# wmtlab/tactileSR

Measured on AMD Instinct MI355X. Metric: SR samples/sec (4x4->40x40), higher is better.
Workload: dtype f32 as 2 power-of-two-scaled fp16 planes x 3 MFMA products, fp32 accumulate (fp32-grade); 1 GPU; tactileSR_model eval forward 4x4->40x40, batch=4096/GPU, fp32 in/out (BASELINE configs[1]); batch_per_gpu=4096, scale_factor=10, seqsCnt=1, parallelism=replicas x1, conv_impl=fp16x3, dist_world_size=1

## Files before the change

### tactilesr_amd/csrc/conv_mfma_k32.hip

```cpp
#include "tsr_common.h"
#include "conv_args.h"
#include "conv_epilogue16.h"
#include "conv_fuse1x1_16.h"
#include "conv_host.h"
#include "tactilesr_hip.h"
#include <type_traits>

typedef _Float16 kf16x8 __attribute__((ext_vector_type(8)));
typedef _Float16 kf16x4 __attribute__((ext_vector_type(4)));

constexpr int k32_row_slots(int px) {
  int rs = px * 4;
  while ((rs & 3) != 2) ++rs;
  return rs;
}

template <int KS, int COUT, int WN, bool DBH = false, int NTHR = 256> struct K32Geom {
  static constexpr int IMG = (NTHR / 64) / WN;
  static constexpr int HH = 8 + KS - 1;
  static constexpr int T = KS * KS;
  static constexpr int HS = (T - 1) / 2;
  static constexpr int PIXB = 64;
  static constexpr int ROWB = k32_row_slots(HH) * 16;
  static constexpr int IMGB = HH * ROWB;
  static constexpr int HALO_B = IMG * IMGB;
  static constexpr int SROWB = k32_row_slots(8) * 16;
  static constexpr int SIMGB = 8 * SROWB;
  static constexpr int SIDE_B = DBH ? 0 : IMG * SIMGB;
  static constexpr int WTAP_B = 2 * 16 * COUT * 2;
  static constexpr int WSLAB_B = 2 * WTAP_B;
  static constexpr int NHB = DBH ? 2 : 1;
  static constexpr int MAIN_LDS = NHB * HALO_B + SIDE_B + 3 * WSLAB_B;
};

constexpr int PAIR_KH[12] = {0, 0, 0, 2, 1, 3, 4, 4, 1, 1, 2, 3};
constexpr int PAIR_KW[12] = {0, 2, 4, 4, 0, 0, 1, 3, 1, 3, 1, 1};
constexpr int PAIR_V[12] = {0, 0, 1, 1, 1, 1, 0, 0, 0, 1, 0, 0};
constexpr int PAIR_OUTER = 8;

template <int KS, int COUT, bool EXT, int WN, bool FUSE2 = false, bool DBH = false, int NTHR = 256, bool PAIR = false>
__global__ __launch_bounds__(NTHR, NTHR == 512 ? 1 : 2) void conv_k32_kernel(const ConvArgs a) {
  static_assert(!PAIR || (KS == 5 && COUT == 128 && !EXT && !FUSE2 && !DBH), "pair form: 5x5 geometry, inference");
  static_assert(COUT == 64 * WN, "every wave owns 64 channels");
  static_assert(!FUSE2 || (!EXT && COUT == 128), "fused 1x1: 128 channels, inference");
  static_assert(NTHR == 256 || (NTHR == 512 && WN == 2), "512 threads: 4 images x 2 C_out halves");
  typedef K32Geom<KS, COUT, WN, DBH, NTHR> G;
  constexpr int NW = NTHR / 64;
  constexpr bool WDMA = !EXT;
  constexpr int IMG = G::IMG, P = KS / 2, HH = G::HH, T = G::T, HS = G::HS, NT = COUT / (16 * WN);
  constexpr int PIXB = G::PIXB, ROWB = G::ROWB, IMGB = G::IMGB, HALO_B = G::HALO_B;
  constexpr int SROWB = G::SROWB, SIMGB = G::SIMGB, SIDE_B = G::SIDE_B;
  constexpr int WTAP_B = G::WTAP_B, WSLAB_B = G::WSLAB_B;
  constexpr int WITEMS = WSLAB_B / 16, WV = (WITEMS + NTHR - 1) / NTHR;
  constexpr int NITEM = IMG * HH * HH * 4, NIT = (NITEM + NTHR - 1) / NTHR;
  constexpr int FUSE_LDS = FUSE2 ? Fuse1x1Geom16<IMG>::BYTES + 64 : 0;
  __shared__ __attribute__((aligned(16))) char lds[G::MAIN_LDS > FUSE_LDS ? G::MAIN_LDS : FUSE_LDS];
  char* halo = lds;
  char* wbuf = lds + G::NHB * HALO_B + SIDE_B;

  const int tid = threadIdx.x;
  const int lane = tid & 63;
  const int wave = tid >> 6;
  const int wave_s = __builtin_amdgcn_readfirstlane(wave);
  const int wm = WN == 2 ? wave >> 1 : wave, wn = WN == 2 ? wave & 1 : 0;
  const int m = lane & 15, g = lane >> 4, khalf = g & 1, tsel = g >> 1;

  float sx = 1.f, accmul = 1.f, sxh = 1.f;
  int bid;
  {
    const int nwg = gridDim.x, q = nwg >> 3, r = nwg & 7;
    const int xcd = blockIdx.x & 7, idx = blockIdx.x >> 3;
    bid = (xcd < r ? xcd * (q + 1) : r * (q + 1) + (xcd - r) * q) + idx;
  }
  const int tpi = a.tiles_x * a.tiles_y;
  const int ig = bid / tpi;
  const int trem = bid - ig * tpi;
  const int ebase = bid * IMG;
  const int ty = trem / a.tiles_x, tx = trem - ty * a.tiles_x;
  const int y0 = ty * 8, x0 = tx * 8, b0 = ig * IMG;
  const int HW = a.H * a.W;
  const int in_blocks = a.in_ctot >> 4;

  int st_src[NIT], st_dst[NIT];
#pragma unroll
  for (int k = 0; k < NIT; ++k) {
    const int it = tid + k * NTHR;
    st_src[k] = -1;
    st_dst[k] = -1;
    if (it < NITEM) {
      const int qd = it & 3, px = it >> 2;
      const int img = px / (HH * HH), rem = px - img * (HH * HH);
      const int hy = rem / HH, hx = rem - hy * HH;
      const int gy = y0 - P + hy, gx = x0 - P + hx, b = b0 + img;
      st_dst[k] = img * IMGB + hy * ROWB + hx * PIXB + qd * 8;
      if (b < a.B && gy >= 0 && gy < a.H && gx >= 0 && gx < a.W)
        st_src[k] = ((img * in_blocks) * HW + gy * a.W + gx) * 16 + qd * 4;
    }
  }
  const float* in_base = a.in + ((size_t)b0 * in_blocks + (a.in_coff >> 4)) * HW * 16;

  const int laneA0 = wm * IMGB + (m >> 3) * ROWB + (m & 7) * PIXB + khalf * 16;
  const int lx = laneA0 + tsel * PIXB;
  constexpr int CK = PAIR ? 3 : KS - 1;
  const int lw = PAIR ? laneA0 + tsel * ROWB
                      : laneA0 + tsel * (ROWB - (KS - 1) * PIXB);
  const int lc = tsel ? laneA0 + CK * ROWB + CK * PIXB
                      : HALO_B + wm * SIMGB + (m >> 3) * SROWB + (m & 7) * PIXB + khalf * 16;
  const int lcs = tsel ? 2 * ROWB : 2 * SROWB;
  const int lcd = laneA0 + (KS - 1) * (ROWB + PIXB) + tsel * HALO_B;
  const int laneB = tsel * WTAP_B + (khalf * COUT + wn * (COUT / WN) + m) * 16;
  const int laneBh = tsel * (WTAP_B / 2) + (khalf * 64 + wn * 32 + m) * 16;

  f32x4 acc[4][NT];
#pragma unroll
  for (int mt = 0; mt < 4; ++mt)
#pragma unroll
    for (int nt = 0; nt < NT; ++nt) acc[mt][nt] = (f32x4){0.f, 0.f, 0.f, 0.f};

  const int nreal = a.cin >> 4;
  const int nchunk = nreal + (nreal & 1);
  const int S = (nchunk >> 1) * T;
  const char* wsrc = (const char*)a.wp;
  const __amdgpu_buffer_rsrc_t wrsrc = __builtin_amdgcn_make_buffer_rsrc((void*)a.wp, 0, 0x7fffffff, 0x00020000);

  f32x4 hsc = {1.f, 1.f, 1.f, 1.f}, hsh = {0.f, 0.f, 0.f, 0.f};
  auto load_halo = [&](int c, f32x4* hv) __attribute__((always_inline)) {
    const float* inc = in_base + (size_t)(c < nreal ? c : nreal - 1) * HW * 16;
    if (EXT && a.in_scale) {
      const int cq = (c < nreal ? c : nreal - 1) * 16 + (tid & 3) * 4;
      hsc = *(const f32x4*)(a.in_scale + cq);
      hsh = *(const f32x4*)(a.in_shift + cq);
    }
#pragma unroll
    for (int k = 0; k < NIT; ++k) hv[k] = *(const f32x4*)(inc + (unsigned)(st_src[k] < 0 ? 0 : st_src[k]));
  };
  auto store_halo = [&](const f32x4* hv, int c, int hb = 0) __attribute__((always_inline)) {
#pragma unroll
    for (int k = 0; k < NIT; ++k) {
      if (st_dst[k] >= 0) {
        f32x4 v = hv[k];
        if (EXT && a.in_scale) {
#pragma unroll
          for (int jj = 0; jj < 4; ++jj) v[jj] = tsr_relu_x2(fmaf(v[jj], hsc[jj], hsh[jj]));
        }
        const bool inside = st_src[k] >= 0 && c < nreal;
#pragma unroll
        for (int jj = 0; jj < 4; ++jj) v[jj] = inside ? v[jj] * sxh : 0.f;
#pragma unroll
        for (int p = 0; p < 2; ++p) {
          kf16x4 bq;
#pragma unroll
          for (int jj = 0; jj < 4; ++jj) {
            bq[jj] = (_Float16)v[jj];
            v[jj] -= (float)bq[jj];
          }
          *(kf16x4*)(halo + hb * HALO_B + st_dst[k] + p * 32) = bq;
        }
      }
    }
  };
#define DMA_BYTES(goff_, slot_, nv_)                                                     \
  {                                                                                      \
    const int vo_ = (int)(goff_) + tid * 16;                                             \
    char* dst_ = wbuf + (slot_) * WSLAB_B + wave_s * 1024;                               \
    _Pragma("unroll") for (int v = 0; v < (nv_); ++v)                                    \
      __builtin_amdgcn_raw_ptr_buffer_load_lds(wrsrc, (__attribute__((address_space(3))) void*)(dst_ + v * NTHR * 16), 16, \
                                               vo_ + v * NTHR * 16, 0, 0, 0);             \
  }
#define LOAD_W(sidx)                                                                     \
  {                                                                                      \
    const f32x4* src_ = (const f32x4*)(wsrc + (size_t)(sidx) * WSLAB_B);                  \
    _Pragma("unroll") for (int v = 0; v < WV; ++v) wreg[v] = src_[tid + v * NTHR];        \
  }
#define STORE_W(slot)                                                                    \
  {                                                                                      \
    char* wb_ = wbuf + (slot) * WSLAB_B;                                                 \
    _Pragma("unroll") for (int v = 0; v < WV; ++v) ((f32x4*)wb_)[tid + v * NTHR] = wreg[v]; \
  }
#define DMA_W(sidx, slot) DMA_BYTES((size_t)(sidx) * WSLAB_B, slot, WV)
#define DMA_WAIT_N(n_) __builtin_amdgcn_s_waitcnt(0x0F70 | ((n_) & 15) | (((n_) >> 4) << 14))
#define DMA_WAIT() DMA_WAIT_N(0)
#define PAIR_HALF(pq_) ((pq_) < 24 && ((pq_) % 12) < PAIR_OUTER)
#define DMA_WP(slot, pq_)                                                                \
  {                                                                                      \
    if (PAIR_HALF(pq_)) { DMA_BYTES(woff, slot, WV / 2); woff += WSLAB_B / 2; }          \
    else { DMA_BYTES(woff, slot, WV); woff += WSLAB_B; }                                 \
  }
#define STEP_BARRIER() __syncthreads()
#define LOAD_A(dst, p_, st_, hb_)                                                        \
  {                                                                                      \
    const int kh_ = PAIR ? PAIR_KH[(st_)] : (2 * (st_)) / KS, kw_ = PAIR ? PAIR_KW[(st_)] : (2 * (st_)) - kh_ * KS; \
    const bool x_ = PAIR ? PAIR_V[(st_)] == 0 : kw_ < KS - 1;                            \
    const char* ab_ = lds + (x_ ? lx : lw) + (hb_) * HALO_B + kh_ * ROWB + kw_ * PIXB + (p_) * 32; \
    _Pragma("unroll") for (int mt = 0; mt < 4; ++mt) dst[mt] = *(const kf16x8*)(ab_ + mt * 2 * ROWB); \
  }
#define LOAD_A_CROSS(dst, p_)                                                            \
  {                                                                                      \
    _Pragma("unroll") for (int mt = 0; mt < 4; ++mt) dst[mt] = *(const kf16x8*)(lds + lc + mt * lcs + (p_) * 32); \
  }
#define LOAD_A_CROSSD(dst, p_)                                                           \
  {                                                                                      \
    _Pragma("unroll") for (int mt = 0; mt < 4; ++mt) dst[mt] = *(const kf16x8*)(lds + lcd + mt * 2 * ROWB + (p_) * 32); \
  }
#define LOAD_B(dst, p_, slot_)                                                           \
  {                                                                                      \
    const char* wb_ = wbuf + (slot_) * WSLAB_B + laneB + (p_) * (2 * COUT * 16);         \
    _Pragma("unroll") for (int nt = 0; nt < NT; ++nt) dst[nt] = *(const kf16x8*)(wb_ + nt * 256); \
  }
#define LOAD_B_HI(dst, p_, slot_)                                                        \
  {                                                                                      \
    const char* wb_ = wbuf + (slot_) * WSLAB_B + laneBh + (p_) * (2 * 64 * 16);          \
    _Pragma("unroll") for (int nt = 2; nt < NT; ++nt) dst[nt] = *(const kf16x8*)(wb_ + (nt - 2) * 256); \
  }
#define MFMA_PHASE_HI(A_, B_)                                                            \
  _Pragma("unroll") for (int mt = 0; mt < 4; ++mt)                                       \
    _Pragma("unroll") for (int nt = 2; nt < NT; ++nt)                                    \
      acc[mt][nt] = __builtin_amdgcn_mfma_f32_16x16x32_f16(A_[mt], B_[nt], acc[mt][nt], 0, 0, 0);
#define MFMA_PHASE(A_, B_)                                                               \
  _Pragma("unroll") for (int mt = 0; mt < 4; ++mt)                                       \
    _Pragma("unroll") for (int nt = 0; nt < NT; ++nt)                                    \
      acc[mt][nt] = __builtin_amdgcn_mfma_f32_16x16x32_f16(A_[mt], B_[nt], acc[mt][nt], 0, 0, 0);
#define INTERLEAVE(n_, per_)                                                             \
  _Pragma("unroll") for (int i_ = 0; i_ < (n_); ++i_) {                                  \
    __builtin_amdgcn_sched_group_barrier(0x008, (per_), 0);                              \
    __builtin_amdgcn_sched_group_barrier(0x100, 1, 0);                                   \
  }

  auto operand_scales = [&]() __attribute__((always_inline)) {
    float mx = a.in_amax ? *a.in_amax : 0.f;
    if (EXT && a.in_scale) {
      __shared__ float bnd[2 * NW];
      float ms = 0.f, mt = 0.f;
      for (int c = threadIdx.x; c < a.cin; c += NTHR) {
        ms = fmaxf(ms, fabsf(a.in_scale[c]));
        mt = fmaxf(mt, fabsf(a.in_shift[c]));
      }
#pragma unroll
      for (int o = 32; o > 0; o >>= 1) {
        ms = fmaxf(ms, __shfl_xor(ms, o));
        mt = fmaxf(mt, __shfl_xor(mt, o));
      }
      if (lane == 0) { bnd[wave * 2] = ms; bnd[wave * 2 + 1] = mt; }
      __syncthreads();
      ms = 0.f; mt = 0.f;
#pragma unroll
      for (int w = 0; w < NW; ++w) { ms = fmaxf(ms, bnd[2 * w]); mt = fmaxf(mt, bnd[2 * w + 1]); }
      mx = mx * ms + mt;
    }
    if (mx > 0.f) {
      int e = (int)((__float_as_uint(mx) >> 23) & 0xFF) - 127;
      int be = 13 - e + 127;
      be = be < 1 ? 1 : (be > 254 ? 254 : be);
      sx = __uint_as_float((unsigned)be << 23);
    }
    float w_inv = a.w_inv_scale;
    if (a.w_amax) {
      const float wmx = *a.w_amax;
      w_inv = 1.f;
      if (wmx > 0.f && wmx < 3.0e38f) {
        int be = 127 - (13 - ((int)((__float_as_uint(wmx) >> 23) & 0xFF) - 127));
        be = be < 1 ? 1 : (be > 254 ? 254 : be);
        w_inv = __uint_as_float((unsigned)be << 23);
      }
    }
    accmul = w_inv / sx;
    sxh = (EXT && a.in_scale) ? 0.5f * sx : sx;
  };

  f32x4 hv[NIT], wreg[WDMA ? 1 : WV];
  size_t woff = 0;
  load_halo(0, hv);
  if constexpr (PAIR) {
    DMA_WP(0, 0);
    DMA_WP(1, 1);
    operand_scales();
  } else if constexpr (WDMA) {
    DMA_W(0, 0);
    if (S > 1) DMA_W(1, 1);
    operand_scales();
  } else {
    LOAD_W(0);
    operand_scales();
    STORE_W(0);
    if (S > 1) { LOAD_W(1); STORE_W(1); }
  }
  store_halo(hv, 0);
  if constexpr (WDMA) { DMA_WAIT(); } else { if (S > 2) LOAD_W(2); }
  __syncthreads();

  kf16x8 A0[4], A1[4], B0[NT] = {}, B1[NT] = {};
  LOAD_A(A1, 1, 0, 0);
  if constexpr (PAIR) { LOAD_B_HI(B0, 0, 0); } else { LOAD_B(B0, 0, 0); }

  constexpr int SCI = IMG * 256 / NTHR, SCS = NTHR / 256;
  const int sc_t = tid & 255, sc_i0 = tid >> 8;
  const int sc_src = sc_i0 * IMGB + ((sc_t >> 5) + CK) * ROWB + (((sc_t >> 2) & 7) + CK) * PIXB + (sc_t & 3) * 16;
  const int sc_dst = HALO_B + sc_i0 * SIMGB + (sc_t >> 5) * SROWB + ((sc_t >> 2) & 7) * PIXB + (sc_t & 3) * 16;

  int s = 0;
  int slot = 0;
  auto block = [&](int c, auto oddc) __attribute__((always_inline)) {
    constexpr int ODD = decltype(oddc)::value;
    constexpr int NST = HS + ODD;
#pragma unroll
    for (int st = 0; st < NST; ++st) {
      const int slot1 = slot == 2 ? 0 : slot + 1;
      const int slot2 = slot1 == 2 ? 0 : slot1 + 1;
      const bool cross = ODD && st == HS;
      f32x4 sidev[SCI];
      if (WDMA && s + 2 < S) {
        if constexpr (PAIR) { DMA_WP(slot2, (ODD * HS + st + 2) % 25); } else { DMA_W(s + 2, slot2); }
      }
      const bool outer = PAIR && st < PAIR_OUTER;
      const bool next_outer = PAIR && (st + 1 < PAIR_OUTER || st + 1 == NST);
      if (cross) { LOAD_A_CROSS(A0, 0); } else { LOAD_A(A0, 0, st, 0); }
      if (outer) { LOAD_B_HI(B1, 1, slot); } else { LOAD_B(B1, 1, slot); }
      if (!ODD && st == 0) {
#pragma unroll
        for (int k = 0; k < SCI; ++k) sidev[k] = *(const f32x4*)(lds + sc_src + k * SCS * IMGB);
      }
      if (st == NST - 2 && c + 1 < nchunk) load_halo(c + 1, hv);
      if (outer) {
        MFMA_PHASE_HI(A1, B0);
        if (!ODD && st == 0) { INTERLEAVE(6 + SCI, 1); } else { INTERLEAVE(6, 1); }
      } else {
        MFMA_PHASE(A1, B0);
        if (!ODD && st == 0) { INTERLEAVE(8 + SCI, 1); } else { INTERLEAVE(8, 2); }
      }
      if (st + 1 < NST) {
        if (ODD && st + 1 == HS) { LOAD_A_CROSS(A1, 1); } else { LOAD_A(A1, 1, st + 1, 0); }
      }
      if (outer) {
        MFMA_PHASE_HI(A0, B0);
        if (st + 1 < NST) { INTERLEAVE(4, 2); }
      } else {
        MFMA_PHASE(A0, B0);
        if (st + 1 < NST) { INTERLEAVE(4, 4); }
      }
      if (next_outer) { LOAD_B_HI(B0, 0, slot1); } else { LOAD_B(B0, 0, slot1); }
      if (outer) {
        MFMA_PHASE_HI(A0, B1);
        if (next_outer) { INTERLEAVE(2, 4); } else { INTERLEAVE(4, 2); }
      } else {
        MFMA_PHASE(A0, B1);
        if (next_outer) { INTERLEAVE(2, 8); } else { INTERLEAVE(4, 4); }
      }
      if (!ODD && st == 0) {
#pragma unroll
        for (int k = 0; k < SCI; ++k) *(f32x4*)(lds + sc_dst + k * SCS * SIMGB) = sidev[k];
      }
      if constexpr (WDMA) {
        if (st == NST - 2 && c + 1 < nchunk) { DMA_WAIT_N(NIT); } else { DMA_WAIT(); }
      } else {
        if (s + 2 < S) STORE_W(slot2);
        if (s + 3 < S) LOAD_W(s + 3);
      }
      STEP_BARRIER();
      if (st + 1 == NST && c + 1 < nchunk) {
        store_halo(hv, c + 1);
        __syncthreads();
        LOAD_A(A1, 1, 0, 0);
      }
      ++s;
      slot = slot1;
    }
  };
  if constexpr (!DBH) {
    for (int c = 0; c < nchunk; c += 2) {
      block(c, std::integral_constant<int, 0>());
      block(c + 1, std::integral_constant<int, 1>());
    }
  } else {
    for (int c = 0; c < nchunk; c += 2) {
#pragma unroll
      for (int p = 0; p < T; ++p) {
        const int slot1 = slot == 2 ? 0 : slot + 1;
        const int slot2 = slot1 == 2 ? 0 : slot1 + 1;
        if (WDMA && s + 2 < S) DMA_W(s + 2, slot2);
        if (p == HS) { LOAD_A_CROSSD(A0, 0); }
        else if (p < HS) { LOAD_A(A0, 0, p, 0); }
        else { LOAD_A(A0, 0, p - HS - 1, 1); }
        LOAD_B(B1, 1, slot);
        if (p == 0) load_halo(c + 1, hv);
        if (p == HS + 1 && c + 2 < nchunk) load_halo(c + 2, hv);
        MFMA_PHASE(A1, B0);
        INTERLEAVE(8, 2);
        if (p + 1 == HS) { LOAD_A_CROSSD(A1, 1); }
        else if (p + 1 < HS) { LOAD_A(A1, 1, p + 1, 0); }
        else if (p + 1 < T) { LOAD_A(A1, 1, p - HS, 1); }
        else { LOAD_A(A1, 1, 0, 0); }
        MFMA_PHASE(A0, B0);
        INTERLEAVE(4, 4);
        LOAD_B(B0, 0, slot1);
        MFMA_PHASE(A0, B1);
        INTERLEAVE(4, 4);
        if (p == HS - 2) store_halo(hv, c + 1, 1);
        if (p == T - 2 && c + 2 < nchunk) store_halo(hv, c + 2, 0);
        if constexpr (WDMA) {
          if (p == 0 || (p == HS + 1 && c + 2 < nchunk)) { DMA_WAIT_N(NIT); } else { DMA_WAIT(); }
        } else {
          if (s + 2 < S) STORE_W(slot2);
          if (s + 3 < S) LOAD_W(s + 3);
        }
        STEP_BARRIER();
        ++s;
        slot = slot1;
      }
    }
  }
#undef DMA_W
#undef LOAD_W
#undef STORE_W
#undef DMA_WP
#undef DMA_BYTES
#undef DMA_WAIT
#undef DMA_WAIT_N
#undef PAIR_HALF
#undef STEP_BARRIER
#undef LOAD_A
#undef LOAD_A_CROSS
#undef LOAD_A_CROSSD
#undef LOAD_B
#undef LOAD_B_HI
#undef MFMA_PHASE_HI
#undef MFMA_PHASE
#undef INTERLEAVE

  if constexpr (FUSE2) conv_fuse1x1_epilogue16<IMG>(a, acc, lds, b0, y0, x0, wm, wn, lane, HW, accmul);
  else conv_epilogue16<COUT, EXT, WN>(a, acc, ebase, b0, y0, x0, wm, wn, lane, HW, accmul);
}

int tsr_conv_k32_images(int cout) { (void)cout; return 4; }

template <int KS, int COUT, bool EXT>
static int launch_k32(const ConvArgs& a, hipStream_t st) {
  constexpr int WN = COUT / 64;
  if constexpr (COUT == 128 && EXT) {
    const int grid = ((a.B + 3) / 4) * a.tiles_x * a.tiles_y;
    hipLaunchKernelGGL((conv_k32_kernel<KS, COUT, EXT, WN, false, KS == 3, 512>), dim3(grid), dim3(512), 0, st, a);
    return tsr_check_launch();
  }
  constexpr int IMG = 4 / WN;
  const int grid = ((a.B + IMG - 1) / IMG) * a.tiles_x * a.tiles_y;
  hipLaunchKernelGGL((conv_k32_kernel<KS, COUT, EXT, WN, false, KS == 3>), dim3(grid), dim3(256), 0, st, a);
  return tsr_check_launch();
}

template <bool EXT> static int dispatch_k32(const ConvArgs& a, int cout, int ks, hipStream_t st) {
  return for_cout_ks(cout, ks, [&](auto CO, auto KS) {
    if constexpr (decltype(KS)::value > 1) return launch_k32<decltype(KS)::value, decltype(CO)::value, EXT>(a, st);
    else return (int)TSR_ERR_ARG;
  });
}
int tsr_conv_k32(const ConvArgs& a, int cout, int ks, bool ext, hipStream_t st) {
  return ext ? dispatch_k32<true>(a, cout, ks, st) : dispatch_k32<false>(a, cout, ks, st);
}

__host__ __device__ inline int pair_logical_channel(int k) {
  const int wn = k >> 6, nt = (k >> 4) & 3, c = k & 15;
  return (nt < 2 ? 0 : 64) + wn * 32 + (nt & 1) * 16 + c;
}
extern "C" int tsr_pair_channel_perm(int* perm128) {
  if (!perm128) return TSR_ERR_ARG;
  for (int k = 0; k < 128; ++k) perm128[k] = pair_logical_channel(k);
  return TSR_OK;
}

__global__ void pack_pair_kernel(const float* __restrict__ w3, const float* __restrict__ w5, _Float16* __restrict__ wp,
                                 int cin, float wscale, const float* __restrict__ w_amax) {
  if (w_amax) {
    const float wm = *w_amax;
    wscale = 1.f;
    if (wm > 0.f && wm < 3.0e38f) {
      int be = 127 + 13 - ((int)((__float_as_uint(wm) >> 23) & 0xFF) - 127);
      be = be < 1 ? 1 : (be > 254 ? 254 : be);
      wscale = __uint_as_float((unsigned)be << 23);
    }
  }
  const int cin_p = (cin + 31) & ~31;
  const size_t total = (size_t)128 * cin_p * 25;
  for (size_t i = blockIdx.x * (size_t)blockDim.x + threadIdx.x; i < total; i += (size_t)gridDim.x * blockDim.x) {
    const int j = i & 7;
    size_t r = i >> 3;
    const int k = r & 127; r >>= 7;
    const int kh2 = r & 1; r >>= 1;
    const int tap = r % 25;
    const int chunk = r / 25;
    const int ci = chunk * 16 + kh2 * 8 + j;
    const int kh = tap / 5, kw = tap - kh * 5;
    const int nt = (k >> 4) & 3, ch = (k >> 6) * 32 + (nt & 1) * 16 + (k & 15);
    float v = 0.f;
    if (ci < cin) {
      if (nt >= 2) v = w5[((size_t)ch * cin + ci) * 25 + tap];
      else if (kh >= 1 && kh <= 3 && kw >= 1 && kw <= 3) v = w3[((size_t)ch * cin + ci) * 9 + (kh - 1) * 3 + (kw - 1)];
    }
    v *= wscale;
    int pos = 24;
#pragma unroll
    for (int st = 0; st < 12; ++st) {
      if (kh == PAIR_KH[st] && kw == PAIR_KW[st]) pos = 2 * st;
      if (kh == PAIR_KH[st] + PAIR_V[st] && kw == PAIR_KW[st] + 1 - PAIR_V[st]) pos = 2 * st + 1;
    }
    const int odd = chunk & 1;
    const bool half = pos < 2 * PAIR_OUTER;
    if (half && nt < 2) continue;
    size_t base = (size_t)(chunk >> 1) * (2 * 65536 + 8192);
    if (pos >= 24) base += 2 * 65536 + (size_t)odd * 4096;
    else if (half) base += (size_t)odd * 65536 + (size_t)(pos >> 1) * 4096 + (size_t)(pos & 1) * 2048;
    else base += (size_t)odd * 65536 + 32768 + (size_t)((pos - 16) >> 1) * 8192 + (size_t)(pos & 1) * 4096;
    const int nch = half ? 64 : 128;
    const int kk = half ? (k >> 6) * 32 + (nt - 2) * 16 + (k & 15) : k;
    for (int p = 0; p < 2; ++p) {
      const _Float16 q = (_Float16)v;
      v -= (float)q;
      wp[base + ((size_t)(p * 2 + kh2) * nch + kk) * 8 + j] = q;
    }
  }
}

extern "C" long long tsr_conv_weight_pair_elems(int cin) { return (long long)(((cin + 31) & ~31) / 32) * (2 * 65536 + 8192); }

extern "C" int tsr_pack_conv_weight_pair_f16s(const float* w3_oihw, const float* w5_oihw, void* w_packed, int cin,
                                              float wscale, const float* w_amax, void* stream) {
  if (!w3_oihw || !w5_oihw || !w_packed || cin <= 0 || (cin & 15) || (!w_amax && !(wscale > 0.f))) return TSR_ERR_ARG;
  hipLaunchKernelGGL(pack_pair_kernel, pack_grid((size_t)128 * ((cin + 31) & ~31) * 25), dim3(256), 0, (hipStream_t)stream,
                     w3_oihw, w5_oihw, (_Float16*)w_packed, cin, wscale, w_amax);
  return tsr_check_launch();
}

extern "C" int tsr_conv2d_fwd_f16s_pair(const float* in, int in_ctot, int in_coff, int cin, const void* w_packed,
                                        float w_inv_scale, const float* in_amax, float* out_amax,
                                        const float* scale, const float* shift, float* out, int out_ctot, int out_coff,
                                        int relu, int B, int H, int W, void* stream) {
  ConvArgs a;
  if (!f16s_scales_ok(in_amax, w_inv_scale) ||
      conv_fill(a, in, in_ctot, in_coff, cin, w_packed, scale, shift, nullptr, 0, 0, out, out_ctot, out_coff, 128, relu, B, H, W))
    return TSR_ERR_ARG;
  a.in_amax = in_amax; a.w_inv_scale = w_inv_scale; a.out_amax = out_amax;
  const int grid = ((B + 1) / 2) * a.tiles_x * a.tiles_y;
  hipLaunchKernelGGL((conv_k32_kernel<5, 128, false, 2, false, false, 256, true>), dim3(grid), dim3(256), 0,
                     (hipStream_t)stream, a);
  return tsr_check_launch();
}

int tsr_conv_k32_fuse1x1(const ConvArgs& a, int ks, hipStream_t st) {
  const int grid = ((a.B + 1) / 2) * a.tiles_x * a.tiles_y;
  if (ks == 5) hipLaunchKernelGGL((conv_k32_kernel<5, 128, false, 2, true>), dim3(grid), dim3(256), 0, st, a);
  else hipLaunchKernelGGL((conv_k32_kernel<3, 128, false, 2, true, true>), dim3(grid), dim3(256), 0, st, a);
  return tsr_check_launch();
}
```

Before: 31830 samples/s.

## Interleave per-row MFMA with split LDS and weight-DMA loads for 5x5 convs

For the non-paired DMA path with 5x5 kernels, the step loop is restructured so each MFMA row is issued alongside individual A/B fragment LDS reads and individual weight DMA pieces, with explicit sched_group_barrier hints per row. The aim is to hide LDS and global-to-LDS latency behind matrix work instead of issuing loads in bulk phases. The buffer resource is also given a tight byte bound instead of a huge range, so the prefetch issued past the last step (it is no longer guarded by s+2<S) reads out of range and returns zero rather than touching memory. This adds scheduling complexity and relies on the bounds check, and the hand-tuned order may hurt if the compiler's own interleave was already better.

```diff
diff --git a/tactilesr_amd/csrc/conv_mfma_k32.hip b/tactilesr_amd/csrc/conv_mfma_k32.hip
--- a/tactilesr_amd/csrc/conv_mfma_k32.hip
+++ b/tactilesr_amd/csrc/conv_mfma_k32.hip
@@ -121,7 +121,8 @@
   const int nchunk = nreal + (nreal & 1);
   const int S = (nchunk >> 1) * T;
   const char* wsrc = (const char*)a.wp;
-  const __amdgpu_buffer_rsrc_t wrsrc = __builtin_amdgcn_make_buffer_rsrc((void*)a.wp, 0, 0x7fffffff, 0x00020000);
+  const int wbytes = !WDMA ? 0x7fffffff : PAIR ? (nchunk >> 1) * ((2 * 65536 + 8192) * 2) : S * WSLAB_B;
+  const __amdgpu_buffer_rsrc_t wrsrc = __builtin_amdgcn_make_buffer_rsrc((void*)a.wp, 0, wbytes, 0x00020000);
 
   f32x4 hsc = {1.f, 1.f, 1.f, 1.f}, hsh = {0.f, 0.f, 0.f, 0.f};
   auto load_halo = [&](int c, f32x4* hv) __attribute__((always_inline)) {
@@ -167,6 +168,9 @@
       __builtin_amdgcn_raw_ptr_buffer_load_lds(wrsrc, (__attribute__((address_space(3))) void*)(dst_ + v * NTHR * 16), 16, \
                                                vo_ + v * NTHR * 16, 0, 0, 0);             \
   }
+#define DMA_PIECE(vo_, slot_, v_)                                                        \
+  __builtin_amdgcn_raw_ptr_buffer_load_lds(wrsrc, (__attribute__((address_space(3))) void*)(wbuf + (slot_) * WSLAB_B + wave_s * 1024 + (v_) * NTHR * 16), \
+                                           16, (vo_) + (v_) * NTHR * 16, 0, 0, 0)
 #define LOAD_W(sidx)                                                                     \
   {                                                                                      \
     const f32x4* src_ = (const f32x4*)(wsrc + (size_t)(sidx) * WSLAB_B);                  \
@@ -187,30 +191,38 @@
     else { DMA_BYTES(woff, slot, WV); woff += WSLAB_B; }                                 \
   }
 #define STEP_BARRIER() __syncthreads()
-#define LOAD_A(dst, p_, st_, hb_)                                                        \
+#define LOAD_A_1(dst, p_, st_, hb_, mt_)                                                 \
   {                                                                                      \
     const int kh_ = PAIR ? PAIR_KH[(st_)] : (2 * (st_)) / KS, kw_ = PAIR ? PAIR_KW[(st_)] : (2 * (st_)) - kh_ * KS; \
     const bool x_ = PAIR ? PAIR_V[(st_)] == 0 : kw_ < KS - 1;                            \
     const char* ab_ = lds + (x_ ? lx : lw) + (hb_) * HALO_B + kh_ * ROWB + kw_ * PIXB + (p_) * 32; \
-    _Pragma("unroll") for (int mt = 0; mt < 4; ++mt) dst[mt] = *(const kf16x8*)(ab_ + mt * 2 * ROWB); \
-  }
+    dst[(mt_)] = *(const kf16x8*)(ab_ + (mt_) * 2 * ROWB);                               \
+  }
+#define LOAD_A(dst, p_, st_, hb_)                                                        \
+  {                                                                                      \
+    _Pragma("unroll") for (int mt = 0; mt < 4; ++mt) LOAD_A_1(dst, p_, st_, hb_, mt);    \
+  }
+#define LOAD_A_CROSS_1(dst, p_, mt_) dst[(mt_)] = *(const kf16x8*)(lds + lc + (mt_) * lcs + (p_) * 32)
 #define LOAD_A_CROSS(dst, p_)                                                            \
   {                                                                                      \
-    _Pragma("unroll") for (int mt = 0; mt < 4; ++mt) dst[mt] = *(const kf16x8*)(lds + lc + mt * lcs + (p_) * 32); \
-  }
+    _Pragma("unroll") for (int mt = 0; mt < 4; ++mt) LOAD_A_CROSS_1(dst, p_, mt);        \
+  }
+#define LOAD_A_CROSSD_1(dst, p_, mt_) dst[(mt_)] = *(const kf16x8*)(lds + lcd + (mt_) * 2 * ROWB + (p_) * 32)
 #define LOAD_A_CROSSD(dst, p_)                                                           \
   {                                                                                      \
-    _Pragma("unroll") for (int mt = 0; mt < 4; ++mt) dst[mt] = *(const kf16x8*)(lds + lcd + mt * 2 * ROWB + (p_) * 32); \
-  }
+    _Pragma("unroll") for (int mt = 0; mt < 4; ++mt) LOAD_A_CROSSD_1(dst, p_, mt);       \
+  }
+#define LOAD_B_1(dst, p_, slot_, nt_)                                                    \
+  dst[(nt_)] = *(const kf16x8*)(wbuf + (slot_) * WSLAB_B + laneB + (p_) * (2 * COUT * 16) + (nt_) * 256)
 #define LOAD_B(dst, p_, slot_)                                                           \
   {                                                                                      \
-    const char* wb_ = wbuf + (slot_) * WSLAB_B + laneB + (p_) * (2 * COUT * 16);         \
-    _Pragma("unroll") for (int nt = 0; nt < NT; ++nt) dst[nt] = *(const kf16x8*)(wb_ + nt * 256); \
-  }
+    _Pragma("unroll") for (int nt = 0; nt < NT; ++nt) LOAD_B_1(dst, p_, slot_, nt);      \
+  }
+#define LOAD_B_HI_1(dst, p_, slot_, nt_)                                                 \
+  dst[(nt_)] = *(const kf16x8*)(wbuf + (slot_) * WSLAB_B + laneBh + (p_) * (2 * 64 * 16) + ((nt_) - 2) * 256)
 #define LOAD_B_HI(dst, p_, slot_)                                                        \
   {                                                                                      \
-    const char* wb_ = wbuf + (slot_) * WSLAB_B + laneBh + (p_) * (2 * 64 * 16);          \
-    _Pragma("unroll") for (int nt = 2; nt < NT; ++nt) dst[nt] = *(const kf16x8*)(wb_ + (nt - 2) * 256); \
+    _Pragma("unroll") for (int nt = 2; nt < NT; ++nt) LOAD_B_HI_1(dst, p_, slot_, nt);   \
   }
 #define MFMA_PHASE_HI(A_, B_)                                                            \
   _Pragma("unroll") for (int mt = 0; mt < 4; ++mt)                                       \
@@ -225,6 +237,28 @@
     __builtin_amdgcn_sched_group_barrier(0x008, (per_), 0);                              \
     __builtin_amdgcn_sched_group_barrier(0x100, 1, 0);                                   \
   }
+
+#define MFMA_ROW(A_, B_, mt_, nt0_)                                                      \
+  _Pragma("unroll") for (int nt = (nt0_); nt < NT; ++nt)                                 \
+    acc[(mt_)][nt] = __builtin_amdgcn_mfma_f32_16x16x32_f16(A_[(mt_)], B_[nt], acc[(mt_)][nt], 0, 0, 0);
+#define HINT_ROW(nm_, nr_, pc_)                                                          \
+  {                                                                                      \
+    if ((nr_) == 2) {                                                                    \
+      __builtin_amdgcn_sched_group_barrier(0x008, (nm_) / 2, 0);                         \
+      __builtin_amdgcn_sched_group_barrier(0x100, 1, 0);                                 \
+      __builtin_amdgcn_sched_group_barrier(0x008, (nm_) - (nm_) / 2, 0);                 \
+      __builtin_amdgcn_sched_group_barrier(0x100, 1, 0);                                 \
+    } else if ((nr_) == 1) {                                                             \
+      __builtin_amdgcn_sched_group_barrier(0x008, (nm_), 0);                             \
+      __builtin_amdgcn_sched_group_barrier(0x100, 1, 0);                                 \
+    } else {                                                                             \
+      __builtin_amdgcn_sched_group_barrier(0x008, (nm_), 0);                             \
+    }                                                                                    \
+    if (pc_) __builtin_amdgcn_sched_group_barrier(0x040, 1, 0);                          \
+    __builtin_amdgcn_sched_barrier(0);                                                   \
+  }
+  constexpr bool WROWS = WDMA && KS == 5 && !PAIR;
+#define PIECE_AT(g_) if ((g_) < WV) DMA_PIECE(vo, slot2, (g_))
 
   auto operand_scales = [&]() __attribute__((always_inline)) {
     float mx = a.in_amax ? *a.in_amax : 0.f;
@@ -308,6 +342,52 @@
       const int slot2 = slot1 == 2 ? 0 : slot1 + 1;
       const bool cross = ODD && st == HS;
       f32x4 sidev[SCI];
+      if constexpr (WROWS) {
+        const int vo = (s + 2) * WSLAB_B + tid * 16;
+        if (st == NST - 2 && c + 1 < nchunk) load_halo(c + 1, hv);
+#pragma unroll
+        for (int mt = 0; mt < 4; ++mt) {
+          MFMA_ROW(A1, B0, mt, 0);
+#pragma unroll
+          for (int h = 0; h < 2; ++h) {
+            if (mt >= 2) { LOAD_B_1(B1, 1, slot, 2 * (mt - 2) + h); }
+            else if (cross) { LOAD_A_CROSS_1(A0, 0, 2 * mt + h); }
+            else { LOAD_A_1(A0, 0, st, 0, 2 * mt + h); }
+          }
+          PIECE_AT(mt);
+          HINT_ROW(4, 2, mt < WV);
+        }
+        if (!ODD && st == 0) {
+#pragma unroll
+          for (int k = 0; k < SCI; ++k) sidev[k] = *(const f32x4*)(lds + sc_src + k * SCS * IMGB);
+          __builtin_amdgcn_sched_group_barrier(0x100, SCI, 0);
+        }
+#pragma unroll
+        for (int mt = 0; mt < 4; ++mt) {
+          MFMA_ROW(A0, B0, mt, 0);
+          if (st + 1 < NST) {
+            if (ODD && st + 1 == HS) { LOAD_A_CROSS_1(A1, 1, mt); } else { LOAD_A_1(A1, 1, st + 1, 0, mt); }
+          }
+          HINT_ROW(4, st + 1 < NST ? 1 : 0, false);
+        }
+        LOAD_B(B0, 0, slot1);
+        MFMA_PHASE(A0, B1);
+        INTERLEAVE(4, 4);
+        if (!ODD && st == 0) {
+#pragma unroll
+          for (int k = 0; k < SCI; ++k) *(f32x4*)(lds + sc_dst + k * SCS * SIMGB) = sidev[k];
+        }
+        DMA_WAIT();
+        STEP_BARRIER();
+        if (st + 1 == NST && c + 1 < nchunk) {
+          store_halo(hv, c + 1);
+          __syncthreads();
+          LOAD_A(A1, 1, 0, 0);
+        }
+        ++s;
+        slot = slot1;
+        continue;
+      }
       if (WDMA && s + 2 < S) {
         if constexpr (PAIR) { DMA_WP(slot2, (ODD * HS + st + 2) % 25); } else { DMA_W(s + 2, slot2); }
       }
@@ -425,6 +505,15 @@
 #undef MFMA_PHASE_HI
 #undef MFMA_PHASE
 #undef INTERLEAVE
+#undef MFMA_ROW
+#undef HINT_ROW
+#undef PIECE_AT
+#undef DMA_PIECE
+#undef LOAD_A_1
+#undef LOAD_A_CROSS_1
+#undef LOAD_A_CROSSD_1
+#undef LOAD_B_1
+#undef LOAD_B_HI_1
 
   if constexpr (FUSE2) conv_fuse1x1_epilogue16<IMG>(a, acc, lds, b0, y0, x0, wm, wn, lane, HW, accmul);
   else conv_epilogue16<COUT, EXT, WN>(a, acc, ebase, b0, y0, x0, wm, wn, lane, HW, accmul);
```

Result: faster. 32300 samples/s (median of 6 runs) (+1.5%).
